# scipr-lab/libiop

Measured on AMD Instinct MI355X. Metric: aurora_prover_fft_field_ops_per_s, higher is better.
Workload: dtype gf2^192 (u32 VALU bit-ops)

## Files before the change

libiop_amd/csrc/fft_add.hip:

```cpp
#include <hip/hip_runtime.h>
#include <cstdlib>
#include <cstring>
#include <map>
#include <memory>
#include <mutex>
#include <vector>
#include "gf192_dev.h"
#include "gf192_host.h"
#include <algorithm>
#include "runtime.h"

namespace iopx {

struct Tuning { int tile_bits, p1_tile_bits, edge_tile_bits, p1_cols, p2_cols, p2_top, comb, p2_threads, p1_fin_tile_bits, p1_fin_cols, small_last, scratch_mb, p1_comb, rs_comb_cap_log2, edge_multi; };
static int env_int(const char *name, int dflt, int lo, int hi) { return opt_range(name, dflt, lo, hi); }
static const Tuning &tuning()
{
    static const Tuning t = [] {
        Tuning u;
        u.tile_bits = env_int("IOPX_TILE_BITS", 11, 4, 12);
        u.p1_tile_bits = (u.tile_bits < 10 ? u.tile_bits : 10);
        u.p1_cols = env_int("IOPX_P1_COLS", 3, 0, u.p1_tile_bits - 3);
        u.p1_fin_tile_bits = (u.tile_bits > u.p1_tile_bits ? u.p1_tile_bits + 1 : u.p1_tile_bits);
        u.p1_fin_cols = (0);
// ... 98 lines not shown
        }
        out[b] = acc;
    }
}

__global__ void k_pad_copy(uint64_t *dst, const uint64_t *src, size_t n_src, size_t n_dst)
{
    for (size_t i = (size_t)blockIdx.x * blockDim.x + threadIdx.x; i < 3 * n_dst; i += (size_t)gridDim.x * blockDim.x) {
        dst[i] = i < 3 * n_src ? src[i] : 0;
    }
}

__global__ void k_fill(uint64_t *dst, const uint64_t *src, int have_src, size_t n)
{
    const uint64_t a = have_src ? src[0] : 0, b = have_src ? src[1] : 0, c = have_src ? src[2] : 0;
    for (size_t i = (size_t)blockIdx.x * blockDim.x + threadIdx.x; i < n; i += (size_t)gridDim.x * blockDim.x) {
        dst[3 * i] = a; dst[3 * i + 1] = b; dst[3 * i + 2] = c;
    }
}

struct P1Params {
    uint64_t *S;
    const uint64_t *pow;
    int d;
    int c, h, A;
    int j0, j1;
    int k_start, k_end;
    int xcd_remap;
    int comb;
    int extra;
    int skip_j0;
};

__device__ __forceinline__ void p1_twist(uint64_t *s, int E, int tid, int nt, const P1Params &p, size_t base, int cmask, int j, bool uniform)
{
    const uint64_t *powj = p.pow + 3 * ((((size_t)2) << p.d) - (((size_t)2) << (p.d - j)));
    if (uniform) {
#pragma unroll 1
        for (int li = tid; li < E; li += nt) {
            const int li_u = (int)__builtin_amdgcn_readfirstlane((uint32_t)(li & ~63));
            const size_t gi_u = base | ((size_t)(li_u >> p.c) << p.h) | (size_t)(li_u & cmask);
            const uint64_t *t = powj + 3 * (gi_u >> j);
            const uint64_t w0 = uniform_load64(t), w1 = uniform_load64(t + 1), w2 = uniform_load64(t + 2);
            gf192 tw;
            tw.w[0] = (uint32_t)w0; tw.w[1] = (uint32_t)(w0 >> 32); tw.w[2] = (uint32_t)w1; tw.w[3] = (uint32_t)(w1 >> 32); tw.w[4] = (uint32_t)w2; tw.w[5] = (uint32_t)(w2 >> 32);
            lds_put(s, E, li, gf_mul_uniform(lds_get(s, E, li), tw));
        }
    } else {
        for (int li = tid; li < E; li += nt) {
            const size_t gi = base | ((size_t)(li >> p.c) << p.h) | (size_t)(li & cmask);
            lds_put(s, E, li, gf_mul(lds_get(s, E, li), gf_load(powj, gi >> j)));
        }
    }
}

__device__ __forceinline__ bool p1_twist_is_uniform(const P1Params &p, int E, int j)
{
    return p.comb && E >= 64 && p.c <= j && j >= p.h + 6 - p.c;
}

template<bool INV>
__global__ void __launch_bounds__(512) k_phase1(P1Params p)
{
    extern __shared__ __attribute__((aligned(16))) uint64_t iopx_smem[];
    uint64_t *s = iopx_smem;
    const int tid = threadIdx.x, nt = blockDim.x;
    const int E = 1 << (p.c + p.A);
    const int midbits = p.h - p.c;
    const size_t o = (p.xcd_remap && (gridDim.x & 7) == 0) ? (size_t)(blockIdx.x & 7) * (gridDim.x >> 3) + (blockIdx.x >> 3) : (size_t)blockIdx.x;
    const size_t mid = o & (((size_t)1 << midbits) - 1), hi = o >> midbits;
    const size_t base = (hi << (p.h + p.A)) | (mid << p.c);
    const int cmask = (1 << p.c) - 1;
    uint64_t *S = p.S + 3 * ((size_t)blockIdx.y << p.d);

    for (int li = tid; li < E; li += nt) {
        const size_t gi = base | ((size_t)(li >> p.c) << p.h) | (size_t)(li & cmask);
        lds_put(s, E, li, gf_load(S, gi));
    }
    __syncthreads();

    const int jb = INV ? p.j1 : p.j0, je = INV ? p.j0 - 1 : p.j1 + 1, js = INV ? -1 : 1;
    for (int j = jb; j != je; j += js) {
        const int ks = (j == p.j0) ? p.k_start : p.d - 2;
        const int ke = (j == p.j1) ? p.k_end : j;
        const bool twist = (ks == p.d - 2) && p.pow && !(p.skip_j0 && j == p.j0);
        if (INV && p.extra >= 0 && j == p.j1 && p.pow) {
            p1_twist(s, E, tid, nt, p, base, cmask, p.extra, p1_twist_is_uniform(p, E, p.extra));
            __syncthreads();
        }
        if (!INV && twist) {
            p1_twist(s, E, tid, nt, p, base, cmask, j, p1_twist_is_uniform(p, E, j));
            __syncthreads();
        }
        const int nops = ks - ke + 1;
        for (int t = 0; t < nops; ++t) {
            const int k = INV ? ke + t : ks - t;
            const int kl = k - p.h + p.c;
            for (int qd = tid; qd < (E >> 2); qd += nt) {
                const int low = qd & ((1 << kl) - 1), high = qd >> kl;
                const int b0 = (high << (kl + 2)) | low;
                const int e1 = b0 | (1 << kl), e2 = b0 | (2 << kl), e3 = b0 | (3 << kl);
                if (!INV) {
                    const gf192 v2 = gf_add(lds_get(s, E, e2), lds_get(s, E, e3));
                    lds_put(s, E, e2, v2);
                    lds_put(s, E, e1, gf_add(lds_get(s, E, e1), v2));
                } else {
                    const gf192 v2 = lds_get(s, E, e2);
                    lds_put(s, E, e1, gf_add(lds_get(s, E, e1), v2));
                    lds_put(s, E, e2, gf_add(v2, lds_get(s, E, e3)));
                }
            }
            __syncthreads();
        }
        if (INV && twist) {
            p1_twist(s, E, tid, nt, p, base, cmask, j, p1_twist_is_uniform(p, E, j));
            __syncthreads();
        }
        if (!INV && p.extra >= 0 && j == p.j1 && p.pow) {
            p1_twist(s, E, tid, nt, p, base, cmask, p.extra, p1_twist_is_uniform(p, E, p.extra));
            __syncthreads();
        }
    }

    for (int li = tid; li < E; li += nt) {
        const size_t gi = base | ((size_t)(li >> p.c) << p.h) | (size_t)(li & cmask);
        gf_store(S, gi, lds_get(s, E, li));
    }
}

struct BfParams {
    const uint64_t *src;
    uint64_t *dst;
    const uint64_t *ltab;
    const uint64_t *rs;
    const uint64_t *rs_comb;
    int src_shared;
    int d, nhi;
    int c, h, A;
    int p_hi, p_lo;
    int a_low, c_top;
    int g_bits;
    size_t total_units;
    size_t coset_base;
    const uint32_t *ltab_small;
    uint32_t rs_small[25];
    int small_k;
    const uint64_t *ltab_small1;
    uint64_t rs_small1[25];
    int small1_k1, small1_k2;
    const uint64_t *rs_tab;
    int rs_tab_groups;
    size_t ncos;
    int cpw;
};

__device__ __forceinline__ gf192 bf_shift_term(const BfParams &p, size_t coset, int l)
{
    if (p.rs_comb) return gf_load(p.rs_comb, coset * p.d + l);
    const size_t gc = p.coset_base + coset;
    gf192 tw = gf_zero();
    if (p.rs_tab) {
        for (int g = 0; g < p.rs_tab_groups; ++g) gf_add_to(tw, gf_load(p.rs_tab, ((size_t)g * 256 + ((gc >> (8 * g)) & 255)) * p.d + l));
        return tw;
    }
    tw = gf_load(p.rs, (size_t)l);
    for (int v = 0; v < p.nhi; ++v) {
        if ((gc >> v) & 1) gf_add_to(tw, gf_load(p.rs, (size_t)(1 + v) * p.d + l));
    }
    return tw;
}

__device__ __forceinline__ gf192 bf_twiddle(const BfParams &p, size_t coset, size_t u, int pbit)
{
    const int l = p.d - 1 - pbit;
    gf192 tw = gf_load(p.ltab, (((size_t)1) << l) - 1 + (u >> (pbit + 1)));
    gf_add_to(tw, bf_shift_term(p, coset, l));
    return tw;
}

__device__ __forceinline__ uint32_t bf_twiddle_small(const BfParams &p, size_t coset, size_t u)
{
    uint32_t y = p.ltab_small[u >> 1] ^ p.rs_small[0];
    const size_t gc = p.coset_base + coset;
    for (int v = 0; v < p.nhi; ++v) {
        if ((gc >> v) & 1) y ^= p.rs_small[1 + v];
    }
    return y;
}

__device__ __forceinline__ uint64_t bf_twiddle_small1(const BfParams &p, size_t coset, size_t u)
{
    uint64_t y = p.ltab_small1[u >> 2] ^ p.rs_small1[0];
    const size_t gc = p.coset_base + coset;
    for (int v = 0; v < p.nhi; ++v) {
        if ((gc >> v) & 1) y ^= p.rs_small1[1 + v];
    }
    return y;
}

__device__ __forceinline__ gf192 bf_twiddle_uniform(const BfParams &p, size_t coset, size_t u_uniform, int pbit)
{
    const int l = p.d - 1 - pbit;
    const uint64_t *t = p.ltab + 3 * ((((size_t)1) << l) - 1 + (u_uniform >> (pbit + 1)));
    uint64_t w0 = uniform_load64(t), w1 = uniform_load64(t + 1), w2 = uniform_load64(t + 2);
    if (p.rs_comb) {
        const uint64_t *r = p.rs_comb + 3 * (coset * p.d + l);
        w0 ^= uniform_load64(r); w1 ^= uniform_load64(r + 1); w2 ^= uniform_load64(r + 2);
    } else {
        const uint64_t *r = p.rs + 3 * (size_t)l;
        w0 ^= uniform_load64(r); w1 ^= uniform_load64(r + 1); w2 ^= uniform_load64(r + 2);
        const size_t gc = p.coset_base + coset;
        for (int v = 0; v < p.nhi; ++v) {
            if ((gc >> v) & 1) {
                const uint64_t *q = p.rs + 3 * ((size_t)(1 + v) * p.d + l);
                w0 ^= uniform_load64(q); w1 ^= uniform_load64(q + 1); w2 ^= uniform_load64(q + 2);
            }
        }
    }
    gf192 tw;
    tw.w[0] = (uint32_t)w0; tw.w[1] = (uint32_t)(w0 >> 32); tw.w[2] = (uint32_t)w1; tw.w[3] = (uint32_t)(w1 >> 32); tw.w[4] = (uint32_t)w2; tw.w[5] = (uint32_t)(w2 >> 32);
    return tw;
}

__global__ void k_rs_combine(uint64_t *out, const uint64_t *rs, int d, int nhi, size_t coset_base, size_t count)
{
    for (size_t e = (size_t)blockIdx.x * blockDim.x + threadIdx.x; e < count; e += (size_t)gridDim.x * blockDim.x) {
        const size_t c = e / d, l = e % d, gc = coset_base + c;
        gf192 acc = gf_load(rs, l);
        for (int v = 0; v < nhi; ++v) {
            if ((gc >> v) & 1) gf_add_to(acc, gf_load(rs, (size_t)(1 + v) * d + l));
        }
        gf_store(out, e, acc);
    }
}

__global__ void k_rs_tables(uint64_t *out, const uint64_t *rs, int d, int nhi, size_t count)
{
    for (size_t e = (size_t)blockIdx.x * blockDim.x + threadIdx.x; e < count; e += (size_t)gridDim.x * blockDim.x) {
        const size_t l = e % d, gb = e / d, b = gb & 255, g = gb >> 8;
        gf192 acc = gf_zero();
        if (g == 0) acc = gf_load(rs, l);
        for (int k = 0; k < 8; ++k) {
            const int v = (int)(8 * g) + k;
            if (v < nhi && ((b >> k) & 1)) gf_add_to(acc, gf_load(rs, (size_t)(1 + v) * d + l));
        }
        gf_store(out, e, acc);
    }
}

template<bool INV, bool COMB, bool LEAN = false>
__device__ __forceinline__ void bf_apply(uint64_t *s, int E, int ia, int ib, const gf192 &tw, bool uniform)
{
    gf192 a = lds_get(s, E, ia), b = lds_get(s, E, ib);
    if (!INV) {
        gf_add_to(a, (COMB && uniform) ? gf_mul_uniform(b, tw) : (LEAN ? gf_mul_lean(b, tw) : gf_mul(b, tw)));
        gf_add_to(b, a);
    } else {
        gf_add_to(b, a);
        gf_add_to(a, (COMB && uniform) ? gf_mul_uniform(b, tw) : (LEAN ? gf_mul_lean(b, tw) : gf_mul(b, tw)));
    }
    lds_put(s, E, ia, a);
    lds_put(s, E, ib, b);
}

template<bool INV>
__device__ __forceinline__ void bf_apply_small(uint64_t *s, int E, int ia, int ib, uint32_t y, int k)
{
    gf192 a = lds_get(s, E, ia), b = lds_get(s, E, ib);
    if (!INV) {
        gf_add_to(a, gf_mul_small_over_xk(b, y, k));
        gf_add_to(b, a);
    } else {
        gf_add_to(b, a);
        gf_add_to(a, gf_mul_small_over_xk(b, y, k));
    }
    lds_put(s, E, ia, a);
    lds_put(s, E, ib, b);
}

template<bool INV>
__device__ __forceinline__ void bf_apply_small1(uint64_t *s, int E, int ia, int ib, uint64_t y, int k1, int k2)
{
    gf192 a = lds_get(s, E, ia), b = lds_get(s, E, ib);
    if (!INV) {
        gf_add_to(a, gf_mul_small2_over(b, (uint32_t)y, (uint32_t)(y >> 32), k1, k2));
        gf_add_to(b, a);
    } else {
        gf_add_to(b, a);
        gf_add_to(a, gf_mul_small2_over(b, (uint32_t)y, (uint32_t)(y >> 32), k1, k2));
    }
    lds_put(s, E, ia, a);
    lds_put(s, E, ib, b);
}

template<bool INV>
__global__ void __launch_bounds__(1024, 1) k_bfly_upper(BfParams p)
{
    extern __shared__ __attribute__((aligned(16))) uint64_t iopx_smem[];
    uint64_t *s = iopx_smem;
    const int tid = threadIdx.x, nt = blockDim.x;
    const int E = 1 << (p.c + p.A);
    const int tpc_bits = p.d - p.c - p.A;
    const size_t unit = blockIdx.x;
    const size_t coset = unit >> tpc_bits, o = unit & (((size_t)1 << tpc_bits) - 1);
    const int midbits = p.h - p.c;
    const size_t mid = o & (((size_t)1 << midbits) - 1), hi = o >> midbits;
    const size_t base = (hi << (p.h + p.A)) | (mid << p.c);
    const int cmask = (1 << p.c) - 1;
    const uint64_t *src = p.src_shared ? p.src : p.src + 3 * (coset << p.d);
    uint64_t *dst = p.dst + 3 * (coset << p.d);

    for (int li = tid; li < E; li += nt) {
        const size_t u = base | ((size_t)(li >> p.c) << p.h) | (size_t)(li & cmask);
        lds_put(s, E, li, gf_load(src, u));
    }
    __syncthreads();

    const int nlev = p.p_hi - p.p_lo + 1;
    for (int t = 0; t < nlev; ++t) {
        const int pbit = INV ? p.p_lo + t : p.p_hi - t;
        const int pl = pbit - p.h + p.c;
        for (int bf = tid; bf < (E >> 1); bf += nt) {
            const int ia = ((bf >> pl) << (pl + 1)) | (bf & ((1 << pl) - 1));
            const gf192 tw = bf_twiddle(p, coset, base | ((size_t)(ia >> p.c) << p.h) | (size_t)(ia & cmask), pbit);
            bf_apply<INV, false>(s, E, ia, ia | (1 << pl), tw, false);
        }
        __syncthreads();
    }

    for (int li = tid; li < E; li += nt) {
        const size_t u = base | ((size_t)(li >> p.c) << p.h) | (size_t)(li & cmask);
        gf_store(dst, u, lds_get(s, E, li));
    }
}

template<bool INV>
__device__ __forceinline__ void bf_apply_io(uint64_t *s, int E, int ia, int ib, const uint64_t *src, uint64_t *dst, size_t ua, size_t ub,
                                            const gf192 &tw, bool from_global, bool to_global)
{
    gf192 a, b;
    if (from_global) { a = gf_load(src, ua); b = gf_load(src, ub); }
    else { a = lds_get(s, E, ia); b = lds_get(s, E, ib); }
    if (!INV) {
        gf_add_to(a, gf_mul_uniform(b, tw));
        gf_add_to(b, a);
    } else {
        gf_add_to(b, a);
        gf_add_to(a, gf_mul_uniform(b, tw));
    }
    if (to_global) { gf_store(dst, ua, a); gf_store(dst, ub, b); }
    else { lds_put(s, E, ia, a); lds_put(s, E, ib, b); }
}

struct UpperOwn { int q, row0; };
__device__ __forceinline__ UpperOwn upper_own(bool inv, int A, int t, int rowset)
{
    if (A == 1) return UpperOwn{0, 0};
    const int te = t & ~1;
    const int r0 = inv ? te : A - 1 - te;
    const bool paired = te + 1 < A;
    UpperOwn o;
    o.q = (inv == paired) ? r0 : r0 - 1;
    o.row0 = ((rowset >> o.q) << (o.q + 2)) | (rowset & ((1 << o.q) - 1));
    return o;
}

template<bool INV>
__global__ void __launch_bounds__(512, 6) k_bfly_upper_comb(BfParams p)
{
    extern __shared__ __attribute__((aligned(16))) uint64_t iopx_smem[];
    uint64_t *s = iopx_smem;
    const int tid = threadIdx.x, nt = blockDim.x;
    const int E = 1 << (p.c + p.A);
    const int tpc_bits = p.d - p.c - p.A;
    const size_t unit = blockIdx.x;
    const size_t coset = unit >> tpc_bits, o = unit & (((size_t)1 << tpc_bits) - 1);
    const int midbits = p.h - p.c;
    const size_t mid = o & (((size_t)1 << midbits) - 1), hi = o >> midbits;
    const size_t base = (hi << (p.h + p.A)) | (mid << p.c);
    const int cmask = (1 << p.c) - 1;
    const uint64_t *src = p.src_shared ? p.src : p.src + 3 * (coset << p.d);
    uint64_t *dst = p.dst + 3 * (coset << p.d);
    const int nlev = p.A;

    const int cbits = p.c - 6;
    const int nitems = nlev == 1 ? (E >> 1) : (E >> 2);
    for (int t0 = 0; t0 < nlev; t0 += 2) {
        const int steps = nlev == 1 ? 1 : 2 * (t0 + 2 <= nlev ? 2 : 1);
        if (t0 > 0) __syncthreads();
#pragma unroll 1
        for (int it = tid; it < nitems; it += nt) {
            const int task = (int)__builtin_amdgcn_readfirstlane((uint32_t)(it >> 6));
            const int col = ((task & ((1 << cbits) - 1)) << 6) | (it & 63);
            const UpperOwn own = upper_own(INV, nlev, t0, task >> cbits);
            gf192 tw = gf_zero();
#pragma unroll 1
            for (int step = 0; step < steps; ++step) {
                const int t = t0 + (step >> 1), k = step & 1;
                const int r = INV ? t : nlev - 1 - t, pbit = p.h + r;
                const int other = (r == own.q) ? own.q + 1 : own.q;
                const int ra = own.row0 | (k << other);
                if (k == 0 || other > r) tw = bf_twiddle_uniform(p, coset, base | ((size_t)ra << p.h), pbit);
                const int ia = (ra << p.c) | col;
                const size_t ua = base | ((size_t)ra << p.h) | (size_t)col;
                bf_apply_io<INV>(s, E, ia, ia | (1 << (r + p.c)), src, dst, ua, ua | ((size_t)1 << pbit), tw, t == 0, t == nlev - 1);
            }
        }
    }
}

template<bool INV, bool COMB>
__global__ void __launch_bounds__(COMB ? 512 : 1024, 1) k_bfly_edge(BfParams p)
{
    extern __shared__ __attribute__((aligned(16))) uint64_t iopx_smem[];
    uint64_t *s = iopx_smem;
    const int tid = threadIdx.x, nt = blockDim.x;
    const int tb = p.a_low + p.c_top;
    const int E = 1 << (tb + p.g_bits);
    const int midbits = p.d - tb;
    const size_t unit0 = (size_t)blockIdx.x << p.g_bits;
    const int lomask = (1 << p.a_low) - 1, tmask = (1 << p.c_top) - 1;

    if (!INV) {
        for (int e = tid; e < E; e += nt) {
            const size_t unit = unit0 + (size_t)(e >> tb);
            if (unit >= p.total_units) continue;
            const size_t coset = unit >> midbits, mid = unit & (((size_t)1 << midbits) - 1);
            const int li = e & ((1 << tb) - 1), top = li >> p.a_low, lo = li & lomask;
            const size_t u = ((size_t)top << (p.d - p.c_top)) | (mid << p.a_low) | (size_t)lo;
            const uint64_t *src = p.src_shared ? p.src : p.src + 3 * (coset << p.d);
            lds_put(s, E, e, gf_load(src, u));
        }
    } else {
        for (int sidx = tid; sidx < E; sidx += nt) {
            const size_t unit = unit0 + (size_t)(sidx >> tb);
            if (unit >= p.total_units) continue;
            const size_t coset = unit >> midbits, mid = unit & (((size_t)1 << midbits) - 1);
            const int tp = sidx & tmask, lo = (sidx >> p.c_top) & lomask;
            const int top = (int)bitrev((uint32_t)tp, p.c_top);
            const size_t v = ((size_t)bitrev((uint32_t)lo, p.a_low) << (p.d - p.a_low)) |
                             ((size_t)bitrev((uint32_t)mid, midbits) << p.c_top) | (size_t)tp;
            const int e = ((sidx >> tb) << tb) | (top << p.a_low) | lo;
            lds_put(s, E, e, gf_load(p.src + 3 * (coset << p.d), v));
        }
    }
    __syncthreads();

    for (int t = 0; t < p.a_low; ++t) {
        const int pbit = INV ? t : p.a_low - 1 - t;
        if (pbit == 0 && p.ltab_small) {
            for (int bf = tid; bf < (E >> 1); bf += nt) {
                const int ia = bf << 1;
                const size_t unit = unit0 + (size_t)(ia >> tb);
                if (unit >= p.total_units) continue;
                const size_t coset = unit >> midbits, mid = unit & (((size_t)1 << midbits) - 1);
                const int li = ia & ((1 << tb) - 1), top = li >> p.a_low, lo = li & lomask;
                const size_t u = ((size_t)top << (p.d - p.c_top)) | (mid << p.a_low) | (size_t)lo;
                bf_apply_small<INV>(s, E, ia, ia | 1, bf_twiddle_small(p, coset, u), p.small_k);
            }
            __syncthreads();
            continue;
        }
        if (pbit == 1 && p.ltab_small1) {
            for (int bf = tid; bf < (E >> 1); bf += nt) {
                const int ia = ((bf >> 1) << 2) | (bf & 1);
                const size_t unit = unit0 + (size_t)(ia >> tb);
                if (unit >= p.total_units) continue;
                const size_t coset = unit >> midbits, mid = unit & (((size_t)1 << midbits) - 1);
                const int li = ia & ((1 << tb) - 1), top = li >> p.a_low, lo = li & lomask;
                const size_t u = ((size_t)top << (p.d - p.c_top)) | (mid << p.a_low) | (size_t)lo;
                bf_apply_small1<INV>(s, E, ia, ia | 2, bf_twiddle_small1(p, coset, u), p.small1_k1, p.small1_k2);
            }
            __syncthreads();
            continue;
        }
        for (int bf = tid; bf < (E >> 1); bf += nt) {
            const int low = bf & ((1 << pbit) - 1), high = bf >> pbit;
            const int ia = (high << (pbit + 1)) | low, ib = ia | (1 << pbit);
            const size_t unit = unit0 + (size_t)(ia >> tb);
            if (unit >= p.total_units) continue;
            const size_t coset = unit >> midbits, mid = unit & (((size_t)1 << midbits) - 1);
            const int li = ia & ((1 << tb) - 1), top = li >> p.a_low, lo = li & lomask;
            const size_t u = ((size_t)top << (p.d - p.c_top)) | (mid << p.a_low) | (size_t)lo;
            bf_apply<INV, COMB>(s, E, ia, ib, bf_twiddle(p, coset, u, pbit), pbit >= 6);
        }
        __syncthreads();
    }

    if (!INV) {
        for (int sidx = tid; sidx < E; sidx += nt) {
            const size_t unit = unit0 + (size_t)(sidx >> tb);
            if (unit >= p.total_units) continue;
            const size_t coset = unit >> midbits, mid = unit & (((size_t)1 << midbits) - 1);
            const int tp = sidx & tmask, lo = (sidx >> p.c_top) & lomask;
            const int top = (int)bitrev((uint32_t)tp, p.c_top);
            const size_t v = ((size_t)bitrev((uint32_t)lo, p.a_low) << (p.d - p.a_low)) |
                             ((size_t)bitrev((uint32_t)mid, midbits) << p.c_top) | (size_t)tp;
            const int e = ((sidx >> tb) << tb) | (top << p.a_low) | lo;
            gf_store(p.dst + 3 * (coset << p.d), v, lds_get(s, E, e));
        }
    } else {
        for (int e = tid; e < E; e += nt) {
            const size_t unit = unit0 + (size_t)(e >> tb);
            if (unit >= p.total_units) continue;
            const size_t coset = unit >> midbits, mid = unit & (((size_t)1 << midbits) - 1);
            const int li = e & ((1 << tb) - 1), top = li >> p.a_low, lo = li & lomask;
            const size_t u = ((size_t)top << (p.d - p.c_top)) | (mid << p.a_low) | (size_t)lo;
            gf_store(p.dst + 3 * (coset << p.d), u, lds_get(s, E, e));
        }
    }
}


template<bool INV>
__global__ void __launch_bounds__(256) k_bfly_edge_multi(BfParams p)
{
    extern __shared__ __attribute__((aligned(16))) uint64_t iopx_smem[];
    const int tid = threadIdx.x, nt = blockDim.x;
    const int tb = p.a_low + p.c_top;
    const int E = 1 << tb, T = 1 << p.c_top;
    const int midbits = p.d - tb;
    const size_t mid = blockIdx.x & (((size_t)1 << midbits) - 1);
    const size_t c0 = (size_t)(blockIdx.x >> midbits) * p.cpw;
    const int lomask = (1 << p.a_low) - 1, tmask = T - 1;
    const int pmin = p.ltab_small ? (p.ltab_small1 ? 2 : 1) : 0;
    const int NTW = pmin < p.a_low ? T * ((1 << (p.a_low - pmin)) - 1) : 0;
    uint64_t *s = iopx_smem;
    uint64_t *tw = s + 3 * E;
    uint64_t *sh = tw + 3 * NTW;
    uint64_t *sm1 = sh + 3 * p.a_low + 2;
    uint32_t *sm0 = (uint32_t *)(sm1 + (p.ltab_small1 ? (E >> 2) : 0));

    for (int pbit = pmin; pbit < p.a_low; ++pbit) {
        const int nb = p.a_low - 1 - pbit, l = p.d - 1 - pbit;
        for (int e = tid; e < (T << nb); e += nt) {
            const size_t blk = ((size_t)(e >> nb) << (p.d - p.c_top - pbit - 1)) | (mid << nb) | (size_t)(e & ((1 << nb) - 1));
            lds_put(tw, NTW, T * ((1 << nb) - 1) + e, gf_load(p.ltab, (((size_t)1) << l) - 1 + blk));
        }
    }
    if (p.ltab_small) {
        for (int e = tid; e < (E >> 1); e += nt) {
            const int top = e >> (p.a_low - 1);
            sm0[e] = p.ltab_small[((size_t)top << (p.d - p.c_top - 1)) | (mid << (p.a_low - 1)) | (size_t)(e & ((1 << (p.a_low - 1)) - 1))];
        }
    }
    if (p.ltab_small1) {
        for (int e = tid; e < (E >> 2); e += nt) {
            const int top = e >> (p.a_low - 2);
            sm1[e] = p.ltab_small1[((size_t)top << (p.d - p.c_top - 2)) | (mid << (p.a_low - 2)) | (size_t)(e & ((1 << (p.a_low - 2)) - 1))];
        }
// ... 400 lines not shown
    const int A = P1_TILE_BITS - P1_COLS;
    const int fin_cols = d <= tuning().p1_fin_tile_bits ? 0 : tuning().p1_fin_cols;
    const int Afin = (d <= tuning().p1_fin_tile_bits ? d : tuning().p1_fin_tile_bits) - fin_cols;
    const int hfin = d - Afin;
    for (int j = 0; j < hfin; ++j) {
        int k = d - 2;
        while (k >= j) {
            if (k + 1 <= P1_TILE_BITS - 1) {
                sched.push_back({0, 0, P1_TILE_BITS, j, j, k, j, -1, 0});
                break;
            }
            const int h = k + 2 - A;
            const int ke = h > j ? h : j;
            sched.push_back({P1_COLS, h, A, j, j, k, ke, -1, 0});
            k = ke - 1;
        }
    }
    sched.push_back({fin_cols, hfin, Afin, hfin, d - 1, d - 2, d - 1, -1, 0});
    if (tuning().comb && tuning().p1_comb) {
        for (size_t i = 0; i + 1 < sched.size(); ++i) {
            P1Pass &a = sched[i], &b = sched[i + 1];
            const bool contiguous_last = a.c == 0 && a.h == 0 && a.j0 == a.j1 && b.j0 == a.j0 + 1 && b.k_start == d - 2;
            if (contiguous_last && b.j0 >= 6) { a.extra = b.j0; b.skip_j0 = 1; }
        }
    }
    return sched;
}

template<bool INV>
static int launch_phase1_pass(const P1Pass &ps, uint64_t *S, const uint64_t *pow, int d_eff, size_t batch)
{
    P1Params p;
    p.S = S;
    p.pow = pow;
    p.d = d_eff; p.c = ps.c; p.h = ps.h; p.A = ps.A;
    p.j0 = ps.j0; p.j1 = ps.j1; p.k_start = ps.k_start; p.k_end = ps.k_end;
    p.xcd_remap = (1);
    p.comb = tuning().comb && tuning().p1_comb;
    p.extra = ps.extra; p.skip_j0 = ps.skip_j0;
    const int tbits = ps.c + ps.A;
    const size_t lds = ((size_t)24) << tbits;
    const size_t blocks = (size_t)1 << (d_eff - tbits);
    const int threads = (1 << tbits) >= 4 * BLOCK_THREADS ? BLOCK_THREADS : ((1 << tbits) >= 256 ? 64 * ((1 << tbits) / 256) : 64);
    int rc = set_lds(k_phase1<INV>, lds);
    if (rc != IOPX_OK) return rc;
    static char names[64][2][40];
    char *nm = names[ps.j0 & 63][ps.k_start == d_eff - 2 ? 1 : 0];
    if (!nm[0]) snprintf(nm, 40, opt("IOPX_PROFILE_LEVELS", 0) ? "k_phase1_%s_L%02d_%s" : "k_phase1_%s", INV ? "inv" : "fwd", ps.j0, ps.k_start == d_eff - 2 ? "tw" : "x");
    { ProfScope ps_(nm, (batch << d_eff) * 48); hipLaunchKernelGGL(k_phase1<INV>, dim3((unsigned)blocks, (unsigned)batch), dim3(threads), lds, stream(), p); }
    return IOPX_OK;
}

__global__ void k_class_extract(const uint64_t *src, uint64_t *dst, int d, int r, size_t cls, size_t batch)
{
    const size_t per = (size_t)1 << (d - r), total = batch * per * 3;
    for (size_t t = (size_t)blockIdx.x * blockDim.x + threadIdx.x; t < total; t += (size_t)gridDim.x * blockDim.x) {
        const size_t w = t % 3, e = t / 3, l = e & (per - 1), b = e >> (d - r);
        dst[t] = src[3 * ((b << d) | (l << r) | cls) + w];
    }
}

__global__ void k_class_merge(const uint64_t *src, uint64_t *dst, int d, int r, size_t batch)
{
    const size_t per = (size_t)1 << (d - r), n = (size_t)1 << d, total = batch * n * 3;
    for (size_t t = (size_t)blockIdx.x * blockDim.x + threadIdx.x; t < total; t += (size_t)gridDim.x * blockDim.x) {
        const size_t w = t % 3, e = t / 3, i = e & (n - 1), b = e >> d, q = i & (((size_t)1 << r) - 1), l = i >> r;
        dst[t] = src[3 * ((q * batch + b) * per + l) + w];
    }
}

extern "C" int iopx_comm_all_gather_dev(iopx_comm *comm, const void *d_send, void *d_recv, size_t bytes_per_rank);

template<bool INV>
static int run_phase1(AddPlan &pl, uint64_t *S, size_t batch = 1)
{
    const int d = pl.d;
    if (d == 0) return IOPX_OK;
    if (!(INV ? pl.have_inv : pl.have_fwd)) {
        int rc = build_pow_tables(pl, INV);
        if (rc != IOPX_OK) return rc;
    }
    const uint64_t *pow = INV ? pl.pow_inv.u64() : pl.pow_fwd.u64();
    std::vector<P1Pass> sched = phase1_schedule(d);
    const int n = (int)sched.size();
    const CommInfo ci = transform_comm();
    int r = 0;
    while ((1 << r) < ci.world) ++r;
    bool split = ci.comm && ci.world > 1 && d >= env_int("IOPX_P1_SHARD_MIN_D", 16, 2, 40) && r < 6 && d - r >= 2;
    for (const P1Pass &ps : sched) if (ps.j0 < r && ps.j1 >= r) split = false;
    if (!split) {
        for (int i = 0; i < n; ++i) {
            int rc = launch_phase1_pass<INV>(sched[INV ? n - 1 - i : i], S, pow, d, batch);
            if (rc != IOPX_OK) return rc;
        }
        IOPX_HIP(hipGetLastError());
        return IOPX_OK;
    }
    const int dt = d - r;
    const size_t per = (size_t)1 << dt;
    const uint64_t *pow_tail = pow + 3 * ((((size_t)2) << d) - (((size_t)2) << dt));
    const std::vector<P1Pass> tail = phase1_schedule(dt);
    TmpBuf cls, all;
    int rc = cls.alloc(batch * per * 24);
    if (rc != IOPX_OK) return rc;
    rc = all.alloc((batch * 24) << d);
    if (rc != IOPX_OK) return rc;
    auto head = [&]() -> int {
        for (int i = 0; i < n; ++i) {
            const P1Pass &ps = sched[INV ? n - 1 - i : i];
            if (ps.j0 >= r) continue;
            int hrc = launch_phase1_pass<INV>(ps, S, pow, d, batch);
            if (hrc != IOPX_OK) return hrc;
        }
        return IOPX_OK;
    };
    if (!INV && (rc = head()) != IOPX_OK) return rc;
    { ProfScope ps_("k_class_extract", batch * per * 48); hipLaunchKernelGGL(k_class_extract, dim3(grid_for(batch * per * 3, 256)), dim3(256), 0, stream(), (const uint64_t *)S, cls.u64(), d, r, (size_t)ci.rank, batch); }
    const int nt = (int)tail.size();
    for (int i = 0; i < nt; ++i) {
        rc = launch_phase1_pass<INV>(tail[INV ? nt - 1 - i : i], cls.u64(), pow_tail, dt, batch);
        if (rc != IOPX_OK) return rc;
    }
    rc = iopx_comm_all_gather_dev(ci.comm, cls.p, all.p, batch * per * 24);
    if (rc != IOPX_OK) return rc;
    { ProfScope ps_("k_class_merge", (batch << d) * 48); hipLaunchKernelGGL(k_class_merge, dim3(grid_for((batch * 3) << d, 256)), dim3(256), 0, stream(), (const uint64_t *)all.u64(), S, d, r, batch); }
    if (INV && (rc = head()) != IOPX_OK) return rc;
    IOPX_HIP(hipGetLastError());
    return IOPX_OK;
}

struct P2Geom { int a_low, c_top; };

#define EDGE_TILE_BITS (tuning().edge_tile_bits)
static P2Geom phase2_geom(int d)
{
    if (d < EDGE_TILE_BITS) return {d, 0};
    return {EDGE_TILE_BITS - P2_TOP, P2_TOP};
}

static void set_small_last(BfParams &p, const AddPlan &pl)
{
    if (!pl.rs_small_ok) return;
    p.ltab_small = (const uint32_t *)pl.ltab_small.p;
    memcpy(p.rs_small, pl.rs_small, sizeof(p.rs_small));
    p.small_k = pl.small_k;
    if (pl.small1_e >= 0) {
        p.ltab_small1 = pl.ltab_small1.u64();
        memcpy(p.rs_small1, pl.rs_small1, sizeof(p.rs_small1));
        p.small1_k1 = pl.small1_e >> 1;
        p.small1_k2 = pl.small1_e - p.small1_k1;
    }
}

template<bool INV>
static int run_phase2(AddPlan &pl, const uint64_t *src, uint64_t *dst, int nhi, size_t coset_begin = 0, size_t coset_count = 0, bool upper_only = false,
                      const uint64_t *shared_rs_comb = nullptr)
{
    const int d = pl.d;
    const P2Geom g = phase2_geom(d);
    const size_t cosets = coset_count ? coset_count : ((size_t)1 << nhi);
    const size_t nd = (size_t)1 << d;
    BfParams p;
    memset(&p, 0, sizeof(p));
    p.ltab = pl.ltab.u64();
    p.rs = pl.rs_cur;
    p.d = d; p.nhi = nhi;
    p.a_low = g.a_low; p.c_top = g.c_top;
    set_small_last(p, pl);
    TmpBuf rs_comb;
    size_t comb_base = 0, comb_count = 0;
    const uint64_t *rs_comb_ptr = shared_rs_comb;
    if (shared_rs_comb) {
        comb_base = coset_begin; comb_count = cosets;
    } else if (!INV && nhi > 0 && cosets * (size_t)d <= ((size_t)1 << tuning().rs_comb_cap_log2)) {
        int rcc = rs_comb.alloc(cosets * d * 24);
        if (rcc != IOPX_OK) return rcc;
        comb_base = coset_begin; comb_count = cosets;
        { ProfScope ps_("k_rs_combine"); hipLaunchKernelGGL(k_rs_combine, dim3(grid_for(cosets * d, 256)), dim3(256), 0, stream(), rs_comb.u64(), pl.rs_cur, d, nhi, coset_begin, cosets * (size_t)d); }
        rs_comb_ptr = rs_comb.u64();
    }
    TmpBuf rs_tab;
    if (!INV && nhi > 0 && !comb_count) {
        const int groups = (nhi + 7) / 8;
        const size_t count = (size_t)groups * 256 * d;
        int rct = rs_tab.alloc(count * 24);
        if (rct != IOPX_OK) return rct;
        { ProfScope ps_("k_rs_combine"); hipLaunchKernelGGL(k_rs_tables, dim3(grid_for(count, 256)), dim3(256), 0, stream(), rs_tab.u64(), pl.rs_cur, d, nhi, count); }
        p.rs_tab = rs_tab.u64();
        p.rs_tab_groups = groups;
    }

    struct Up { int h, A, c; };
    std::vector<Up> ups;
    {
        int top = d;
        while (top > g.a_low) {
            int A = TILE_BITS - P2_COLS;
            if (top - A < g.a_low) A = top - g.a_low;
            const int c = TILE_BITS - A > g.a_low ? g.a_low : TILE_BITS - A;
            ups.push_back({top - A, A, c});
            top -= A;
        }
    }
    const int tb = g.a_low + g.c_top;

    auto launch_edge = [&](const uint64_t *s, uint64_t *dd, int shared, size_t ncos, size_t cbase) -> int {
        int g_bits = EDGE_TILE_BITS - tb;
        const size_t units = ncos << (d - tb);
        while (g_bits > 0 && ((size_t)1 << g_bits) > units) --g_bits;
        const size_t lds = ((size_t)24) << (tb + g_bits);
        const size_t blocks = (units + ((size_t)1 << g_bits) - 1) >> g_bits;
        const int elems = 1 << (tb + g_bits);
        const int maxt = (256);
        const int threads = elems >= 4 * maxt ? maxt : (elems >= 256 ? elems / 4 : 64);
        p.src = s; p.dst = dd; p.src_shared = shared;
        p.g_bits = g_bits; p.total_units = units; p.coset_base = cbase;
        p.rs_comb = comb_count ? rs_comb_ptr + 3 * (cbase - comb_base) * d : nullptr;
        int rc;
        const int pmin = p.ltab_small ? (p.ltab_small1 ? 2 : 1) : 0;
        const size_t ntw = pmin < p.a_low ? ((size_t)1 << p.c_top) * (((size_t)1 << (p.a_low - pmin)) - 1) : 0;
        const size_t lds_m = lds + 24 * ntw + 8 * (3 * (size_t)p.a_low + 2) + (p.ltab_small1 ? 8 * ((size_t)elems >> 2) : 0) + (p.ltab_small ? 4 * ((size_t)elems >> 1) : 0);
        if (tuning().edge_multi > 0 && g_bits == 0 && tb == EDGE_TILE_BITS && threads <= 256 && lds_m <= 80 * 1024) {
            size_t cpw = (size_t)tuning().edge_multi < ncos ? (size_t)tuning().edge_multi : ncos;
            cpw = (ncos + (ncos + cpw - 1) / cpw - 1) / ((ncos + cpw - 1) / cpw);
            p.ncos = ncos; p.cpw = (int)cpw;
            const size_t blocks_m = ((ncos + cpw - 1) / cpw) << (d - tb);
            if ((rc = set_lds(k_bfly_edge_multi<INV>, lds_m)) != IOPX_OK) return rc;
            { ProfScope ps_(INV ? "k_bfly_edge_inv" : "k_bfly_edge_fwd", (ncos << d) * 48, ((ncos << d) >> 1) * (size_t)p.a_low); hipLaunchKernelGGL((k_bfly_edge_multi<INV>), dim3((unsigned)blocks_m), dim3(threads), lds_m, stream(), p); }
            return IOPX_OK;
        }
        if ((rc = set_lds(k_bfly_edge<INV, false>, lds)) != IOPX_OK) return rc;
        { ProfScope ps_(INV ? "k_bfly_edge_inv" : "k_bfly_edge_fwd", (ncos << d) * 48, ((ncos << d) >> 1) * (size_t)p.a_low); hipLaunchKernelGGL((k_bfly_edge<INV, false>), dim3((unsigned)blocks), dim3(threads), lds, stream(), p); }
        return IOPX_OK;
    };
    auto launch_upper = [&](const Up &u, const uint64_t *s, uint64_t *dd, int shared, size_t ncos, size_t cbase) -> int {
        p.src = s; p.dst = dd; p.src_shared = shared;
        p.c = u.c; p.h = u.h; p.A = u.A;
        p.p_hi = u.h + u.A - 1; p.p_lo = u.h;
        const int tbits = u.c + u.A;
        const size_t lds = ((size_t)24) << tbits;
        const size_t blocks = ncos << (d - tbits);
        p.total_units = blocks; p.coset_base = cbase;
        p.rs_comb = comb_count ? rs_comb_ptr + 3 * (cbase - comb_base) * d : nullptr;
        const int maxt = (tuning().comb && u.c < 6) ? 1024 : tuning().p2_threads;
        int threads = (1 << tbits) >= 2 * maxt ? maxt : ((1 << tbits) >= 128 ? (1 << tbits) / 2 : 64);
        int rc;
        if (tuning().comb && u.c >= 6) {
            if (u.A >= 2) threads = std::max(64, std::min(512, (1 << tbits) / 4));
            if ((rc = set_lds(k_bfly_upper_comb<INV>, lds)) != IOPX_OK) return rc;
            { ProfScope ps_(INV ? "k_bfly_upper_inv" : "k_bfly_upper_fwd", (ncos << d) * 48, ((ncos << d) >> 1) * (size_t)u.A); hipLaunchKernelGGL((k_bfly_upper_comb<INV>), dim3((unsigned)blocks), dim3(threads), lds, stream(), p); }
        } else {
            if ((rc = set_lds(k_bfly_upper<INV>, lds)) != IOPX_OK) return rc;
            { ProfScope ps_(INV ? "k_bfly_upper_inv" : "k_bfly_upper_fwd", (ncos << d) * 48, ((ncos << d) >> 1) * (size_t)u.A); hipLaunchKernelGGL((k_bfly_upper<INV>), dim3((unsigned)blocks), dim3(threads), lds, stream(), p); }
        }
        return IOPX_OK;
    };

    int rc;
    if (INV) {
        rc = launch_edge(src, dst, 0, cosets, 0);
        if (rc != IOPX_OK) return rc;
        for (size_t i = ups.size(); i-- > 0; ) {
            rc = launch_upper(ups[i], dst, dst, 0, cosets, 0);
            if (rc != IOPX_OK) return rc;
        }
    } else if (ups.empty()) {
        rc = launch_edge(src, dst, 1, cosets, coset_begin);
        if (rc != IOPX_OK) return rc;
    } else if (nhi == 0) {
        uint64_t *W = const_cast<uint64_t *>(src);
        for (size_t i = 0; i < ups.size(); ++i) {
            rc = launch_upper(ups[i], W, W, 1, 1, 0);
            if (rc != IOPX_OK) return rc;
        }
        rc = launch_edge(W, dst, 1, 1, 0);
        if (rc != IOPX_OK) return rc;
    } else if (upper_only) {
        for (size_t i = 0; i < ups.size(); ++i) {
            rc = launch_upper(ups[i], i == 0 ? src : dst, dst, i == 0 ? 1 : 0, cosets, coset_begin);
            if (rc != IOPX_OK) return rc;
        }
    } else {
        size_t group = SCRATCH_BYTES / (nd * 24);
        if (group < 1) group = 1;
        if (group > cosets) group = cosets;
        group = (cosets + (cosets + group - 1) / group - 1) / ((cosets + group - 1) / group);
        TmpBuf scratch;
        rc = scratch.alloc(group * nd * 24);
        if (rc != IOPX_OK) return rc;
        for (size_t c0 = 0; c0 < cosets; c0 += group) {
            const size_t nc = cosets - c0 < group ? cosets - c0 : group;
            for (size_t i = 0; i < ups.size(); ++i) {
                rc = launch_upper(ups[i], i == 0 ? src : scratch.u64(), scratch.u64(), i == 0 ? 1 : 0, nc, coset_begin + c0);
                if (rc != IOPX_OK) return rc;
            }
            rc = launch_edge(scratch.u64(), dst + 3 * c0 * nd, 0, nc, coset_begin + c0);
            if (rc != IOPX_OK) return rc;
        }
    }
    IOPX_HIP(hipGetLastError());
    return IOPX_OK;
}


static int run_phase2_fwd_batch(AddPlan &pl, const uint64_t *const *srcs, uint64_t *const *dsts, size_t batch, int nhi, size_t coset_begin, size_t coset_count)
{
    const int d = pl.d;
    const size_t cosets = coset_count ? coset_count : ((size_t)1 << nhi);
    const bool batched_edge = tuning().comb && env_int("IOPX_EDGE_BATCH", 1, 0, 1) && batch >= 2 && batch <= 4 && nhi > 0 && d >= EDGE_TILE_BITS + 1 &&
                              cosets * (size_t)d <= ((size_t)1 << tuning().rs_comb_cap_log2);
    if (!batched_edge) {
        for (size_t k = 0; k < batch; ++k) {
            const int rc = run_phase2<false>(pl, srcs[k], dsts[k], nhi, coset_begin, coset_count);
            if (rc != IOPX_OK) return rc;
        }
        return IOPX_OK;
    }
    const size_t nd = (size_t)1 << d;
    size_t group = SCRATCH_BYTES / (nd * 24);
    if (group < 1) group = 1;
    if (group > cosets) group = cosets;
    group = (cosets + (cosets + group - 1) / group - 1) / ((cosets + group - 1) / group);
    std::vector<std::unique_ptr<TmpBuf>> scratch;
    for (size_t k = 0; k < batch; ++k) {
        scratch.emplace_back(new TmpBuf());
        const int rc = scratch.back()->alloc(group * nd * 24);
        if (rc != IOPX_OK) return rc;
    }
    TmpBuf rs_comb;
    {
        const int rc = rs_comb.alloc(cosets * d * 24);
        if (rc != IOPX_OK) return rc;
        ProfScope ps_("k_rs_combine");
        hipLaunchKernelGGL(k_rs_combine, dim3(grid_for(cosets * d, 256)), dim3(256), 0, stream(), rs_comb.u64(), pl.rs_cur, d, nhi, coset_begin, cosets * (size_t)d);
    }
    for (size_t c0 = 0; c0 < cosets; c0 += group) {
        const size_t nc = cosets - c0 < group ? cosets - c0 : group;
        for (size_t k = 0; k < batch; ++k) {
            const int rc = run_phase2<false>(pl, srcs[k], scratch[k]->u64(), nhi, coset_begin + c0, nc, true, rs_comb.u64() + 3 * c0 * d);
            if (rc != IOPX_OK) return rc;
        }
        const P2Geom g = phase2_geom(d);
        BfBatchParams q;
        memset(&q, 0, sizeof(q));
        BfParams &p = q.p;
        p.ltab = pl.ltab.u64(); p.rs = pl.rs_cur; p.d = d; p.nhi = nhi;
        p.a_low = g.a_low;
        set_small_last(p, pl);
        p.c_top = batch == 4 ? g.c_top - 1 : g.c_top;
        p.g_bits = 0;
        const int tb = p.a_low + p.c_top;
        p.total_units = nc << (d - tb);
        p.coset_base = coset_begin + c0;
        int rc;
        p.rs_comb = rs_comb.u64() + 3 * c0 * d;
        q.batch = (int)batch;
        for (size_t k = 0; k < batch; ++k) { q.srcs[k] = scratch[k]->u64(); q.dsts[k] = dsts[k] + 3 * c0 * nd; }
        const size_t lds = (((size_t)24) << tb) * batch;
        if ((rc = set_lds(k_bfly_edge_fwd_batch, lds)) != IOPX_OK) return rc;
        ProfScope ps_("k_bfly_edge_fwd_batch", batch * (nc << d) * 48, batch * ((nc << d) >> 1) * (size_t)p.a_low);
        hipLaunchKernelGGL(k_bfly_edge_fwd_batch, dim3((unsigned)p.total_units), dim3(512), lds, stream(), q);
    }
    IOPX_HIP(hipGetLastError());
    return IOPX_OK;
}

static int check_basis_args(const uint64_t *basis, size_t m, const uint64_t *shift)
{
    if (m > 40) return fail(IOPX_ERR_INVALID_ARGUMENT, "domain dimension %zu too large", m);
    if ((m > 0 && !basis) || !shift) return fail(IOPX_ERR_INVALID_ARGUMENT, "null basis/shift");
    return IOPX_OK;
}

}

using namespace iopx;

extern "C" {

int iopx_clear_plans(void)
{
    std::lock_guard<std::mutex> lk(g_plan_mu);
    (void)hipDeviceSynchronize();
    g_plans.clear();
    clear_mul_plans();
    clear_dist_plans();
    clear_poseidon_sets();
    clear_gf64_plans();
    clear_gf128_plans();
    clear_domain_tables();
    tmp_trim();
    return IOPX_OK;
}

int iopx_add_lde_gf192_dev(const uint64_t *d_coeffs, size_t n_coeffs, const uint64_t *basis, size_t m,
                           const uint64_t *shift, size_t coset_begin, size_t coset_count, uint64_t *d_out)
{
    int rc = ensure_device();
    if (rc != IOPX_OK) return rc;
    rc = check_basis_args(basis, m, shift);
    if (rc != IOPX_OK) return rc;
    const size_t n = (size_t)1 << m;
    if (n_coeffs > n) return fail(IOPX_ERR_INVALID_ARGUMENT, "additive FFT: %zu coefficients exceed the domain size %zu", n_coeffs, n);
    if (!d_out || (n_coeffs && !d_coeffs)) return fail(IOPX_ERR_INVALID_ARGUMENT, "null buffer");
    const int d = n_coeffs <= 1 ? 0 : (int)ceil_log2(n_coeffs);
    const int nhi = (int)m - d;
    const size_t all_cosets = (size_t)1 << nhi;
    if (coset_count == 0 || coset_begin >= all_cosets || coset_count > all_cosets - coset_begin)
        return fail(IOPX_ERR_INVALID_ARGUMENT, "coset range [%zu, +%zu) outside the %zu cosets of the transform", coset_begin, coset_count, all_cosets);
    if (n_coeffs <= 1) {
        { ProfScope ps_("k_fill"); hipLaunchKernelGGL(k_fill, dim3(grid_for(coset_count, 256)), dim3(256), 0, stream(), d_out, d_coeffs, (int)(n_coeffs == 1), coset_count); }
        IOPX_HIP(hipGetLastError());
        return IOPX_OK;
    }
    AddPlan *pl = nullptr;
    rc = get_plan(basis, d, &pl);
    if (rc != IOPX_OK) return rc;
    rc = upload_rs(*pl, hgf192::from_words(shift), basis + 3 * (size_t)d, nhi);
    if (rc != IOPX_OK) return rc;

    const size_t nd = (size_t)1 << d;
    TmpBuf work;
    rc = work.alloc(nd * 24);
    if (rc != IOPX_OK) return rc;
    uint64_t *W = work.u64();
    { ProfScope ps_("k_pad_copy"); hipLaunchKernelGGL(k_pad_copy, dim3(grid_for(3 * nd, 256)), dim3(256), 0, stream(), W, d_coeffs, n_coeffs, nd); }
    rc = run_phase1<false>(*pl, W);
    if (rc != IOPX_OK) return rc;
    rc = run_phase2<false>(*pl, W, d_out, nhi, coset_begin, coset_count);
    if (rc != IOPX_OK) return rc;
    return IOPX_OK;
}

int iopx_add_fft_gf192_dev(const uint64_t *d_coeffs, size_t n_coeffs, const uint64_t *basis, size_t m,
                           const uint64_t *shift, uint64_t *d_out)
{
    if (m > 40) return fail(IOPX_ERR_INVALID_ARGUMENT, "domain dimension %zu too large", m);
    const size_t n = (size_t)1 << m;
    if (n_coeffs > n) return fail(IOPX_ERR_INVALID_ARGUMENT, "additive FFT: %zu coefficients exceed the domain size %zu", n_coeffs, n);
    const int d = n_coeffs <= 1 ? 0 : (int)ceil_log2(n_coeffs);
    return iopx_add_lde_gf192_dev(d_coeffs, n_coeffs, basis, m, shift, 0, (size_t)1 << ((int)m - d), d_out);
}

int iopx_add_ifft_gf192_dev(const uint64_t *d_evals, const uint64_t *basis, size_t m, const uint64_t *shift,
                            uint64_t *d_out)
{
    int rc = ensure_device();
    if (rc != IOPX_OK) return rc;
    rc = check_basis_args(basis, m, shift);
    if (rc != IOPX_OK) return rc;
    if (!d_evals || !d_out) return fail(IOPX_ERR_INVALID_ARGUMENT, "null buffer");
    if (m == 0) {
        { const int crc_ = iopx::copy_d2d(d_out, d_evals, 24); if (crc_ != IOPX_OK) return crc_; }
        return IOPX_OK;
    }
    AddPlan *pl = nullptr;
    rc = get_plan(basis, (int)m, &pl);
    if (rc != IOPX_OK) return rc;
    rc = upload_rs(*pl, hgf192::from_words(shift), nullptr, 0);
    if (rc != IOPX_OK) return rc;
    const uint64_t *src = d_evals;
    TmpBuf tmp;
    if (d_evals == d_out) {
        rc = tmp.alloc(((size_t)24) << m);
        if (rc != IOPX_OK) return rc;
        { const int crc_ = iopx::copy_d2d(tmp.p, d_evals, ((size_t)24) << m); if (crc_ != IOPX_OK) return crc_; }
        src = tmp.u64();
    }
    rc = run_phase2<true>(*pl, src, d_out, 0);
    if (rc != IOPX_OK) return rc;
    rc = run_phase1<true>(*pl, d_out);
    if (rc != IOPX_OK) return rc;
    return IOPX_OK;
}

int iopx_add_ifft_gf192_batch_dev(const uint64_t *d_evals, size_t batch, const uint64_t *basis, size_t m, const uint64_t *shift,
                                  uint64_t *d_out)
{
    int rc = ensure_device();
    if (rc != IOPX_OK) return rc;
    rc = check_basis_args(basis, m, shift);
    if (rc != IOPX_OK) return rc;
    if (!d_evals || !d_out) return fail(IOPX_ERR_INVALID_ARGUMENT, "null buffer");
    if (batch == 0 || batch > 65535) return fail(IOPX_ERR_INVALID_ARGUMENT, "batch size %zu outside 1..65535", batch);
    const size_t bytes = (batch * 24) << m;
    if (m == 0) {
        { const int crc_ = iopx::copy_d2d(d_out, d_evals, bytes); if (crc_ != IOPX_OK) return crc_; }
        return IOPX_OK;
    }
    AddPlan *pl = nullptr;
    rc = get_plan(basis, (int)m, &pl);
    if (rc != IOPX_OK) return rc;
// ... 405 lines not shown
```

Before: 1557 billion.

## Precompute shared top-level butterfly products across cosets in forward additive FFT

Adds a precompute kernel that, for the top butterfly level of the forward transform, multiplies the shared source upper half by a small set of basis twiddle combinations (linear in the coset index bits). The upper comb kernel then reconstructs each coset's top-level product by XOR-summing a few precomputed terms instead of doing a field multiplication per element. It also optionally remaps block-to-coset order so blocks sharing the same term data run together for cache reuse. This trades GF(2^192) multiplies for extra global loads and a temporary buffer sized by the number of coset-bit terms.

```diff
diff --git a/libiop_amd/csrc/fft_add.hip b/libiop_amd/csrc/fft_add.hip
--- a/libiop_amd/csrc/fft_add.hip
+++ b/libiop_amd/csrc/fft_add.hip
@@ -274,7 +274,54 @@
     int rs_tab_groups;
     size_t ncos;
     int cpw;
+    const uint64_t *top_terms;
+    int top_wa, top_wb, top_nvar;
+    int top_remap;
 };
+
+struct TopShared {
+    const uint64_t *terms = nullptr;
+    int wa = 0, wb = 0, nvar = 0;
+    int remap = 0;
+};
+struct TopTermsParams {
+    const uint64_t *src, *ltab, *rs;
+    uint64_t *out;
+    int d, wa, wb, nvar, chunk;
+    size_t fixed;
+};
+
+__global__ void __launch_bounds__(256) k_bfly_upper_fwd_terms(TopTermsParams q)
+{
+    const size_t half = (size_t)1 << (q.d - 1);
+    const size_t cpv = half / (size_t)q.chunk;
+    const size_t k = blockIdx.x / cpv, u0 = (blockIdx.x % cpv) * (size_t)q.chunk;
+    const size_t na = (size_t)1 << q.wa, nb = (size_t)(q.wb - q.wa);
+    const bool first = k < na;
+    const size_t bits = first ? (q.fixed | k) : (k < na + nb ? (size_t)1 << (q.wa + (int)(k - na)) : (k - na - nb + 1) << q.wb);
+    gf192 m = gf_zero();
+    if (first) { m = gf_load(q.ltab, 0); gf_add_to(m, gf_load(q.rs, 0)); }
+    for (int v = 0; (bits >> v) != 0; ++v) {
+        if ((bits >> v) & 1) gf_add_to(m, gf_load(q.rs, (size_t)(1 + v) * q.d));
+    }
+    for (int li = threadIdx.x; li < q.chunk; li += blockDim.x) {
+        const size_t u = u0 + (size_t)li;
+        gf_store(q.out, k * half + u, gf_mul_uniform(gf_load(q.src, half + u), m));
+    }
+}
+
+__device__ __forceinline__ gf192 bf_top_sum(const BfParams &p, size_t gc, size_t u)
+{
+    const size_t half = (size_t)1 << (p.d - 1);
+    gf192 acc = gf_load(p.top_terms, (gc & (((size_t)1 << p.top_wa) - 1)) * half + u);
+    size_t k = (size_t)1 << p.top_wa;
+    for (int v = p.top_wa; v < p.top_wb; ++v, ++k) {
+        if ((gc >> v) & 1) gf_add_to(acc, gf_load(p.top_terms, k * half + u));
+    }
+    const size_t j = (gc >> p.top_wb) & (((size_t)1 << (p.top_nvar - p.top_wb)) - 1);
+    if (j) gf_add_to(acc, gf_load(p.top_terms, (k + j - 1) * half + u));
+    return acc;
+}
 
 __device__ __forceinline__ gf192 bf_shift_term(const BfParams &p, size_t coset, int l)
 {
@@ -474,6 +521,17 @@
     else { lds_put(s, E, ia, a); lds_put(s, E, ib, b); }
 }
 
+__device__ __forceinline__ void bf_apply_top(const BfParams &p, size_t gc, uint64_t *s, int E, int ia, int ib, const uint64_t *src, uint64_t *dst,
+                                             size_t ua, size_t ub, bool to_global)
+{
+    gf192 a = gf_load(src, ua);
+    gf_add_to(a, bf_top_sum(p, gc, ua));
+    gf192 b = gf_load(src, ub);
+    gf_add_to(b, a);
+    if (to_global) { gf_store(dst, ua, a); gf_store(dst, ub, b); }
+    else { lds_put(s, E, ia, a); lds_put(s, E, ib, b); }
+}
+
 struct UpperOwn { int q, row0; };
 __device__ __forceinline__ UpperOwn upper_own(bool inv, int A, int t, int rowset)
 {
@@ -487,16 +545,22 @@
     return o;
 }
 
-template<bool INV>
+template<bool INV, bool TOP = false>
 __global__ void __launch_bounds__(512, 6) k_bfly_upper_comb(BfParams p)
 {
+    static_assert(!(INV && TOP), "the shared top level is the forward transform's");
     extern __shared__ __attribute__((aligned(16))) uint64_t iopx_smem[];
     uint64_t *s = iopx_smem;
     const int tid = threadIdx.x, nt = blockDim.x;
     const int E = 1 << (p.c + p.A);
     const int tpc_bits = p.d - p.c - p.A;
     const size_t unit = blockIdx.x;
-    const size_t coset = unit >> tpc_bits, o = unit & (((size_t)1 << tpc_bits) - 1);
+    size_t coset = unit >> tpc_bits, o = unit & (((size_t)1 << tpc_bits) - 1);
+    if (TOP && p.top_remap) {
+        const size_t ncos = p.total_units >> tpc_bits, j = unit >> 3;
+        coset = j % ncos;
+        o = ((j / ncos) << 3) | (unit & 7);
+    }
     const int midbits = p.h - p.c;
     const size_t mid = o & (((size_t)1 << midbits) - 1), hi = o >> midbits;
     const size_t base = (hi << (p.h + p.A)) | (mid << p.c);
@@ -516,8 +580,17 @@
             const int col = ((task & ((1 << cbits) - 1)) << 6) | (it & 63);
             const UpperOwn own = upper_own(INV, nlev, t0, task >> cbits);
             gf192 tw = gf_zero();
+            if (TOP && t0 == 0) {
+                const int r = nlev - 1, other = (r == own.q) ? own.q + 1 : own.q;
+                for (int k = 0; k < (nlev == 1 ? 1 : 2); ++k) {
+                    const int ra = own.row0 | (k << other);
+                    const int ia = (ra << p.c) | col;
+                    const size_t ua = base | ((size_t)ra << p.h) | (size_t)col;
+                    bf_apply_top(p, p.coset_base + coset, s, E, ia, ia | (1 << (r + p.c)), src, dst, ua, ua | ((size_t)1 << (p.h + r)), nlev == 1);
+                }
+            }
 #pragma unroll 1
-            for (int step = 0; step < steps; ++step) {
+            for (int step = (TOP && t0 == 0) ? 2 : 0; step < steps; ++step) {
                 const int t = t0 + (step >> 1), k = step & 1;
                 const int r = INV ? t : nlev - 1 - t, pbit = p.h + r;
                 const int other = (r == own.q) ? own.q + 1 : own.q;
@@ -1224,9 +1297,59 @@
     }
 }
 
+struct Up { int h, A, c; };
+static std::vector<Up> upper_passes(int d)
+{
+    const P2Geom g = phase2_geom(d);
+    std::vector<Up> ups;
+    int top = d;
+    while (top > g.a_low) {
+        int A = TILE_BITS - P2_COLS;
+        if (top - A < g.a_low) A = top - g.a_low;
+        const int c = TILE_BITS - A > g.a_low ? g.a_low : TILE_BITS - A;
+        ups.push_back({top - A, A, c});
+        top -= A;
+    }
+    return ups;
+}
+
+static int make_top_terms(AddPlan &pl, const uint64_t *src, int nhi, size_t coset_begin, size_t cosets, TmpBuf &buf, TopShared &ts)
+{
+    ts = TopShared();
+    const int mode = opt("IOPX_TOP_SHARED", 1);
+    const int d = pl.d;
+    if (mode <= 0 || !tuning().comb || nhi == 0 || cosets < 2) return IOPX_OK;
+    const std::vector<Up> ups = upper_passes(d);
+    if (ups.empty() || ups[0].c < 6) return IOPX_OK;
+    const size_t diff = coset_begin ^ (coset_begin + cosets - 1);
+    int nvar = 0;
+    while (nvar < 63 && (diff >> nvar) != 0) ++nvar;
+    if (2 * (size_t)(1 + nvar) > cosets) return IOPX_OK;
+    int wa = 0, wb = nvar;
+    size_t nvec = (size_t)(1 + nvar);
+    ts.remap = mode <= 2;
+    if (mode == 2 || mode == 4) {
+        const int ta = nvar < 3 ? nvar : 3;
+        const size_t tvec = ((size_t)1 << ta) + ((size_t)1 << (nvar - ta)) - 1;
+        if (2 * tvec <= cosets) { wa = wb = ta; nvec = tvec; }
+    }
+    const size_t half = (size_t)1 << (d - 1);
+    int rc = buf.alloc(nvec * half * 24);
+    if (rc != IOPX_OK) return rc;
+    TopTermsParams q;
+    q.src = src; q.ltab = pl.ltab.u64(); q.rs = pl.rs_cur; q.out = buf.u64();
+    q.d = d; q.wa = wa; q.wb = wb; q.nvar = nvar;
+    q.chunk = half < 256 ? (int)half : 256;
+    q.fixed = (coset_begin >> nvar) << nvar;
+    const size_t blocks = nvec * (half / (size_t)q.chunk);
+    { ProfScope ps_("k_bfly_upper_fwd_terms", (1 + nvec) * half * 24, nvec * half); hipLaunchKernelGGL(k_bfly_upper_fwd_terms, dim3((unsigned)blocks), dim3(q.chunk), 0, stream(), q); }
+    ts.terms = buf.u64(); ts.wa = wa; ts.wb = wb; ts.nvar = nvar;
+    return IOPX_OK;
+}
+
 template<bool INV>
 static int run_phase2(AddPlan &pl, const uint64_t *src, uint64_t *dst, int nhi, size_t coset_begin = 0, size_t coset_count = 0, bool upper_only = false,
-                      const uint64_t *shared_rs_comb = nullptr)
+                      const uint64_t *shared_rs_comb = nullptr, const TopShared *shared_top = nullptr)
 {
     const int d = pl.d;
     const P2Geom g = phase2_geom(d);
@@ -1262,17 +1385,13 @@
         p.rs_tab_groups = groups;
     }
 
-    struct Up { int h, A, c; };
-    std::vector<Up> ups;
-    {
-        int top = d;
-        while (top > g.a_low) {
-            int A = TILE_BITS - P2_COLS;
-            if (top - A < g.a_low) A = top - g.a_low;
-            const int c = TILE_BITS - A > g.a_low ? g.a_low : TILE_BITS - A;
-            ups.push_back({top - A, A, c});
-            top -= A;
-        }
+    const std::vector<Up> ups = upper_passes(d);
+    TmpBuf top_buf;
+    TopShared top;
+    if (shared_top) top = *shared_top;
+    else if (!INV && !upper_only) {
+        const int rct = make_top_terms(pl, src, nhi, coset_begin, cosets, top_buf, top);
+        if (rct != IOPX_OK) return rct;
     }
     const int tb = g.a_low + g.c_top;
 
@@ -1307,6 +1426,10 @@
     };
     auto launch_upper = [&](const Up &u, const uint64_t *s, uint64_t *dd, int shared, size_t ncos, size_t cbase) -> int {
         p.src = s; p.dst = dd; p.src_shared = shared;
+        const bool top_shared = !INV && shared && top.terms && u.h + u.A == d;
+        p.top_terms = top_shared ? top.terms : nullptr;
+        p.top_wa = top.wa; p.top_wb = top.wb; p.top_nvar = top.nvar;
+        p.top_remap = top.remap && d - u.c - u.A >= 3;
         p.c = u.c; p.h = u.h; p.A = u.A;
         p.p_hi = u.h + u.A - 1; p.p_lo = u.h;
         const int tbits = u.c + u.A;
@@ -1319,6 +1442,11 @@
         int rc;
         if (tuning().comb && u.c >= 6) {
             if (u.A >= 2) threads = std::max(64, std::min(512, (1 << tbits) / 4));
+            if (top_shared) {
+                if ((rc = set_lds(k_bfly_upper_comb<false, true>, lds)) != IOPX_OK) return rc;
+                { ProfScope ps_("k_bfly_upper_fwd", (ncos << d) * 48, ((ncos << d) >> 1) * (size_t)(u.A - 1)); hipLaunchKernelGGL((k_bfly_upper_comb<false, true>), dim3((unsigned)blocks), dim3(threads), lds, stream(), p); }
+                return IOPX_OK;
+            }
             if ((rc = set_lds(k_bfly_upper_comb<INV>, lds)) != IOPX_OK) return rc;
             { ProfScope ps_(INV ? "k_bfly_upper_inv" : "k_bfly_upper_fwd", (ncos << d) * 48, ((ncos << d) >> 1) * (size_t)u.A); hipLaunchKernelGGL((k_bfly_upper_comb<INV>), dim3((unsigned)blocks), dim3(threads), lds, stream(), p); }
         } else {
@@ -1406,10 +1534,17 @@
         ProfScope ps_("k_rs_combine");
         hipLaunchKernelGGL(k_rs_combine, dim3(grid_for(cosets * d, 256)), dim3(256), 0, stream(), rs_comb.u64(), pl.rs_cur, d, nhi, coset_begin, cosets * (size_t)d);
     }
+    std::vector<std::unique_ptr<TmpBuf>> top_bufs;
+    std::vector<TopShared> tops(batch);
+    for (size_t k = 0; k < batch; ++k) {
+        top_bufs.emplace_back(new TmpBuf());
+        const int rc = make_top_terms(pl, srcs[k], nhi, coset_begin, cosets, *top_bufs.back(), tops[k]);
+        if (rc != IOPX_OK) return rc;
+    }
     for (size_t c0 = 0; c0 < cosets; c0 += group) {
         const size_t nc = cosets - c0 < group ? cosets - c0 : group;
         for (size_t k = 0; k < batch; ++k) {
-            const int rc = run_phase2<false>(pl, srcs[k], scratch[k]->u64(), nhi, coset_begin + c0, nc, true, rs_comb.u64() + 3 * c0 * d);
+            const int rc = run_phase2<false>(pl, srcs[k], scratch[k]->u64(), nhi, coset_begin + c0, nc, true, rs_comb.u64() + 3 * c0 * d, &tops[k]);
             if (rc != IOPX_OK) return rc;
         }
         const P2Geom g = phase2_geom(d);
```

New measurement: 1571 billion (median of 6 runs). No clear change (+0.9%).
